# sashajenner/honours

Hardware: AMD Instinct MI355X
Metric: raw-signal MB/s (compress+decompress) (higher is better)
Workload: dtype u16

## Files before the change

honours_amd/csrc/press_huffman.hip:

```cpp

#include "press_internal.h"
#include "press_packed.h"
#include <cstddef>
#include <type_traits>

namespace ph {

#ifdef HUF_STAMPS
__device__ unsigned long long g_hstamp[32];
#define HSTAMP_DECL                                             \
	unsigned long long hs_t = __builtin_amdgcn_s_memtime(); \
	unsigned long long hs_acc[8] = { 0, 0, 0, 0, 0, 0, 0, 0 }
#define HSTAMP(i)                                                              \
	do {     \
		__builtin_amdgcn_sched_barrier(0);                             \
		const unsigned long long hs_n = __builtin_amdgcn_s_memtime(); \
		hs_acc[(i) & 7] += hs_n - hs_t;                                \
		hs_t = hs_n;                                                   \
		__builtin_amdgcn_sched_barrier(0);                             \
	} while (0)
#define HSTAMP_FLUSH(base)                                                     \
	do {                                                                   \
		if ((threadIdx.x & 63) == 0)                                   \
			for (int hs_i = 0; hs_i < 8; hs_i++)                   \
// ... 54 lines not shown
	typedef uint32_t u32x4_u __attribute__((ext_vector_type(4), aligned(1)));
	const u32x4_u v = __builtin_nontemporal_load(reinterpret_cast<const u32x4_u *>(p));
	return make_uint4(v.x, v.y, v.z, v.w);
}
__device__ __forceinline__ uint32_t ld4_pay(const uint8_t *p)
{
	typedef uint32_t __attribute__((aligned(1))) u32_u;
	return __builtin_nontemporal_load(reinterpret_cast<const u32_u *>(p));
}
#else
__device__ __forceinline__ uint4 ld16_pay(const uint8_t *p)
{
	uint4 v;
	__builtin_memcpy(&v, p, 16);
	return v;
}
__device__ __forceinline__ uint32_t ld4_pay(const uint8_t *p)
{
	uint32_t v;
	__builtin_memcpy(&v, p, 4);
	return v;
}
#endif

template <int NDW, int S = 64>
__device__ __forceinline__ void col_load(uint32_t *col, const uint8_t *src, int32_t rb0, int32_t lo, int32_t nby)
{
	if (rb0 >= lo && rb0 + 4 * NDW <= nby) {
		const uint8_t *q = src + rb0;
		uint4 t[NDW / 4 ? NDW / 4 : 1];
		uint32_t x[NDW % 4 ? NDW % 4 : 1];
#pragma unroll
		for (int j = 0; j < NDW / 4; j++)
			t[j] = ld16_pay(q + 16 * j);
#pragma unroll
		for (int j = 0; j < NDW % 4; j++)
			x[j] = ld4_pay(q + 4 * (NDW / 4 * 4 + j));
#pragma unroll
		for (int j = 0; j < NDW / 4; j++) {
			col[(4 * j + 0) * S] = t[j].x;
			col[(4 * j + 1) * S] = t[j].y;
			col[(4 * j + 2) * S] = t[j].z;
			col[(4 * j + 3) * S] = t[j].w;
		}
#pragma unroll
		for (int j = 0; j < NDW % 4; j++)
			col[(NDW / 4 * 4 + j) * S] = x[j];
	} else if (nby > lo) {
		uint8_t b[4 * NDW];
#pragma unroll
		for (int i = 0; i < 4 * NDW; i++) {
			const int32_t r = rb0 + i;
			b[i] = src[r < lo ? lo : (r >= nby ? nby - 1 : r)];
		}
#pragma unroll
		for (int j = 0; j < NDW; j++) {
			uint32_t x = 0;
#pragma unroll
			for (int i = 0; i < 4; i++) {
				const int32_t r = rb0 + 4 * j + i;
				x |= (r >= lo && r < nby) ? (uint32_t) b[4 * j + i] << (8 * i) : 0u;
			}
			col[j * S] = x;
		}
	} else {
#pragma unroll
		for (int j = 0; j < NDW; j++)
			col[j * S] = 0;
	}
}

__device__ __forceinline__ int32_t unzz8(uint32_t z) { return (int32_t) (z >> 1) ^ -(int32_t) (z & 1u); }

typedef __attribute__((address_space(3))) const uint32_t *lds_cu32p;
typedef __attribute__((address_space(3))) const uint16_t *lds_cu16p;
typedef __attribute__((address_space(3))) const uint8_t *lds_cu8p;
typedef __attribute__((address_space(3))) uint8_t *lds_u8p;

struct LenTabs {
	alignas(16) uint32_t alut[1 << HUF_LUT_BITS];
	alignas(16) uint16_t flut[1 << HUF_LUT_BITS];
	alignas(16) uint16_t l2ld[HUF_L2_ENTRIES];
};

template <bool TRIE, int S = 64>
__device__ __forceinline__ uint32_t len_scan(const uint32_t *col_, const LenTabs *tabs, const HuffDev *hd, uint32_t start,
					     uint32_t lim, uint32_t nb, uint32_t &cnt, uint32_t &dsum)
{
	const lds_cu32p col = (lds_cu32p) col_;
	const lds_cu32p alut = (lds_cu32p) tabs->alut;
	const lds_cu16p flut = (lds_cu16p) tabs->flut;
	const lds_cu16p l2ld = (lds_cu16p) tabs->l2ld;
	bool bad = start == HEND;
	uint32_t L = lim < nb ? lim : nb;
	if (bad)
		L = 0;
	auto long_ld = [&](uint32_t e, uint32_t wnd) -> uint32_t {
		if (TRIE && e == 0xFFFFFFFFu) {
			const uint32_t t = trie_code(hd, wnd);
			return t ? (((t >> 24) & 31u) | (((uint32_t) unzz8(t & 0xFFu) & 0xFFu) << 8)) : 0u;
		}
		const uint32_t v = l2ld[(e & 0xFFFu) + ((wnd >> HUF_LUT_BITS) & ((1u << ((e >> 12) & 15u)) - 1u))];
		return v == 0xFFFFu ? 0u : v;
	};
	constexpr uint32_t PB = 30;
	const lds_cu32p colm = col - S;
	uint32_t A = (bad ? 0u : start) + PB;
	{
		int32_t LmP = (int32_t) L - HUF_LUT_BITS + (int32_t) PB;
		uint32_t jj = (A >> 5) & 15u;
		uint32_t w0 = colm[__umul24(jj, (uint32_t) S)], w1 = colm[__umul24(jj, (uint32_t) S) + S];
		while ((int32_t) (A & 0x1FFu) <= LmP) {
			const uint32_t pp = A & 0x1FFu;
			{
				const uint32_t w2 = colm[__umul24(jj, (uint32_t) S) + 2 * S];
				const uint32_t wnd = __builtin_amdgcn_alignbit(w1, w0, A);
				const uint32_t e = *(lds_cu32p) ((lds_cu8p) alut + (wnd & (((1u << HUF_LUT_BITS) - 1u) << 2)));
				uint32_t inc = e;
				if ((int32_t) e < 0) {
					const uint32_t ld = long_ld(e, wnd >> 2);
					const uint32_t tot = ld & 0xFFu;
					inc = tot | (1u << HUF_A_CNT) | (((uint32_t) (int32_t) (int8_t) (ld >> 8) & 0x7FFFu) << HUF_A_SUM);
					if (tot - 1u >= L + PB - pp) {
						inc = 0;
						LmP = -1;
					}
				}
				A += inc;
				const uint32_t jn = (A >> 5) & 15u;
				if (jn != jj) {
					w0 = w1;
					w1 = w2;
				}
				jj = jn;
			}
		}
	}
	uint32_t p = (A & 0x1FFu) - PB;
	uint32_t c = (A >> HUF_A_CNT) & 0x7Fu;
	int32_t d = (int32_t) (A << 1) >> 17;
	for (;;) {
		const bool act = p < L;
		if (!any64(act))
			break;
		const uint32_t pp = act ? p : 0u;
		const uint32_t j = pp >> 5;
		const int r0 = (int) __umul24(j, (uint32_t) S);
		const uint32_t wnd = __builtin_amdgcn_alignbit(col[r0 + S], col[r0], pp);
		const uint32_t e = alut[wnd & ((1u << HUF_LUT_BITS) - 1u)];
		const uint32_t f = flut[wnd & ((1u << HUF_LUT_BITS) - 1u)];
		uint32_t tot = e & 15u, n = (e >> HUF_A_CNT) & 15u, len1 = f & 0xFFu;
		int32_t dall = (int32_t) (e << 1) >> 17, d1 = (int32_t) (int8_t) (f >> 8);
		bool fail = false;
		if (any64(act && (int32_t) e < 0)) {
			if (act && (int32_t) e < 0) {
				const uint32_t ld = long_ld(e, wnd);
				tot = len1 = ld & 0xFFu;
				dall = d1 = (int32_t) (int8_t) (ld >> 8);
				fail = tot == 0;
				n = 1;
			}
		}
		const bool fits = pp + tot <= L;
		const bool cut = !fits && pp + len1 > nb;
		if (act && !fail && !cut) {
			p += fits ? tot : len1;
			c += fits ? n : 1u;
			d += fits ? dall : d1;
		}
		if (act && (fail || cut)) {
			bad = true;
			L = 0;
		}
	}
	cnt = c;
	dsum = (uint32_t) d & 0xFFFFu;
	return bad ? HEND : (p >= nb && p < lim ? HEND : p);
}

__device__ __forceinline__ void wave_lds_sync()
{
	__builtin_amdgcn_fence(__ATOMIC_RELEASE, "wavefront");
	__builtin_amdgcn_wave_barrier();
	__builtin_amdgcn_fence(__ATOMIC_ACQUIRE, "wavefront");
}



#ifndef HUF_SYNC_PER_CU
#define HUF_SYNC_PER_CU 2
#endif
#ifndef HUF_RUNUP_EIGHTHS
#define HUF_RUNUP_EIGHTHS 4
#endif
constexpr int WGS = 1024;
constexpr int SYNC_S = 64;

__device__ __forceinline__ uint32_t pack_rec(uint32_t f, uint32_t c, uint32_t d)
{
	return (f == HEND ? R_END : f) | ((c & 0xFFu) << 8) | ((d & 0xFFFFu) << 16);
}

constexpr uint32_t LIST_NONE = 0xFFFFFFFFu;
constexpr uint32_t SYNC_UC = 16;

__device__ __forceinline__ void list_push(uint32_t *list, uint32_t *cnt, uint32_t cap, bool yes, uint32_t value, uint32_t lane)
{
	const unsigned long long m = __ballot(yes);
// ... 336 lines not shown
		if (e < nex)
			val[e] = z | (((xcum + before + inc - dl) & 0xFFFFu) << 16);
		xcum += total;
		__syncthreads();
	}
	__syncthreads();
	const uint64_t cumall = s_cum;
	const uint32_t nlow = cumall < want ? (uint32_t) cumall : want;
	const bool fused = nlow >= 1 && (nex == 0 || pos[nex - 1] < nlow + nex);
	const uint32_t zd0 = uniform(a.meta[r].zd0) & 0xFFFFu, q = uniform(a.meta[r].q);
	const uint64_t src0 = a.htiles[k0].src;
	const int64_t nby0 = (int64_t) ((a.htiles[k0].nbits + 7u) >> 3);
	uint64_t cum = 0;
	uint32_t dcum = 0;
	for (uint32_t b = 0; b < nu; b += HT) {
		const uint32_t u = b + tid;
		uint32_t c = 0, dt = 0;
		if (u < nu) {
			const uint2 w = hw[u];
			c = w.x;
			dt = w.y & 0xFFFFu;
		}
		const uint32_t inc = wave_scan(c);
		const uint32_t dinc = wave_scan(dt);
		if ((tid & 63) == 63) {
			s_w[tid >> 6] = inc;
			s_wd[tid >> 6] = dinc;
		}
		__syncthreads();
		uint32_t before = 0, total = 0, dbefore = 0, dtotal = 0;
#pragma unroll
		for (int w2 = 0; w2 < HT / 64; w2++) {
			const uint32_t x = s_w[w2], y = s_wd[w2];
			if (w2 < (int) (tid >> 6)) {
				before += x;
				dbefore += y;
			}
			total += x;
			dtotal += y;
		}
		if (u < nu) {
			const uint64_t ob = cum + before + inc - c;
			const uint32_t L0 = ob > 0xFFFFFFFFull ? 0xFFFFFFFFu : (uint32_t) ob;
			const uint32_t quota = L0 >= want ? 0u : (c < want - L0 ? c : want - L0);
			const uint32_t L1 = L0 + quota;
			uint32_t Ea = 0, Eb = 0;
			if (fused && quota) {
				keys_below2(pos, nex, L0, L1, Ea, Eb);
				if (L1 == nlow)
					Eb = nex;
			}
			uint32_t bz = zd0;
			if (L0) {
				bz = unzz16(zd0) + ((dcum + dbefore + dinc - dt) & 0xFFFFu);
				if (Ea) {
					const uint32_t pv = val[Ea - 1];
					bz += (pv >> 16) + unzz16(pv & 0xFFFFu);
				}
				bz &= 0xFFFFu;
			}
			const uint64_t src = src0 + (uint64_t) u * UB;
			const int64_t nby = nby0 - (int64_t) u * UB;
			const uint32_t nbyc = nby <= 0 ? 0u : (nby > (int64_t) HUF_U_NBY ? HUF_U_NBY : (uint32_t) nby);
			uint4 *d = reinterpret_cast<uint4 *>(a.hunit + (uint64_t) k0 * UPT + u);
			d[0] = make_uint4((uint32_t) src, (uint32_t) (src >> 32) | (bz << 16), (uint32_t) o0, (uint32_t) (o0 >> 32));
			d[1] = make_uint4(L0, quota | (nbyc << 14) | ((q & 15u) << 26) | (fused ? 1u << 30 : 0u), Ea, Eb - Ea);
		}
		cum += total;
		dcum += dtotal;
		__syncthreads();
	}
	static_assert(HUF_U_QUOTA >= 64u * 255u, "a unit's quota");
	if (tid == 0) {
		a.meta[r].nlow = nlow;
		if (fused)
			a.hread[2 * r + 1] = nt | HUF_FUSED;
	}
}


constexpr uint32_t EMIT_STG = 4096;

template <bool TRIE>
__device__ __forceinline__ void emit_codes(const uint32_t *col_, const uint32_t *lut_, const uint16_t *lut2_,
					   const HuffDev *hd, uint32_t p, uint32_t nmine, uint8_t *wp_)
{
	const lds_cu32p col = (lds_cu32p) col_;
	const lds_cu8p lut = (lds_cu8p) lut_;
	const lds_cu16p lut2 = (lds_cu16p) lut2_;
	auto long_entry = [&](uint32_t e, uint32_t wnd) -> uint32_t {
		if (TRIE && e == 0xFFFFFFFFu) {
			const uint32_t t = trie_code(hd, wnd);
			return t ? ((t & 0xFFFFFF00u) | ((uint32_t) unzz8(t & 0xFFu) & 0xFFu)) : 0u;
		}
		const uint32_t e2 = lut2[(e & 0xFFFu) + ((wnd >> HUF_LUT_BITS) & ((1u << ((e >> 12) & 15u)) - 1u))];
		return e2 == 0xFFFFu ? 0u : (((uint32_t) unzz8(e2 & 0xFFu) & 0xFFu) | (e2 & 0x1F00u) | ((e2 & 0x1F00u) << 16));
	};
	typedef lds_u8p WP;
	WP w = (WP) wp_;
	const WP wend = w + nmine;
	WP wlim = nmine ? wend - 1 : w;
	constexpr uint32_t PB = 30;
	const lds_cu32p colm = col - 64;
	uint32_t pp = p + PB;
	uint32_t jj = pp >> 5;
	uint32_t w0 = colm[__umul24(jj, 64u)], w1 = colm[__umul24(jj, 64u) + 64];
	while (w < wlim) {
		{
			const uint32_t w2 = colm[__umul24(jj, 64u) + 128];
			const uint32_t wnd = __builtin_amdgcn_alignbit(w1, w0, pp);
			uint32_t e = *(lds_cu32p) (lut + (wnd & (((1u << HUF_LUT_BITS) - 1u) << 2)));
			if (e >= HUF_LONG)
				e = long_entry(e, wnd >> 2);
			w[0] = (uint8_t) e;
			w[1] = (uint8_t) (e >> 16);
			w += 1u + ((e >> 29) & 1u);
			pp += (e >> 8) & 0x1Fu;
			const uint32_t jn = pp >> 5;
			if (jn != jj) {
				w0 = w1;
				w1 = w2;
			}
			jj = jn;
		}
	}
	if (w < wend) {
		const uint32_t wnd = __builtin_amdgcn_alignbit(w1, w0, pp);
		uint32_t e = *(lds_cu32p) (lut + (wnd & (((1u << HUF_LUT_BITS) - 1u) << 2)));
		if (e >= HUF_LONG)
			e = long_entry(e, wnd >> 2);
		w[0] = (uint8_t) e;
	}
}


__device__ __forceinline__ uint32_t lower_bound_u32(const uint32_t *p, uint32_t n, uint32_t key)
{
	uint32_t lo = 0, hi = n;
	while (lo < hi) {
		const uint32_t mid = (lo + hi) >> 1;
		if (p[mid] < key)
			lo = mid + 1;
		else
			hi = mid;
	}
	return lo;
}

template <typename LOWAT>
__device__ __forceinline__ void gather8(LOWAT lowat, const uint32_t *pos, const uint32_t *val, uint32_t zd0,
					uint32_t i0, uint32_t Ia, uint32_t Ib, uint32_t e_first, uint32_t e_cnt,
					uint32_t v[4])
{
	v[0] = v[1] = v[2] = v[3] = 0;
	const uint32_t lo = i0 > Ia ? i0 : Ia;
	const uint32_t hi = i0 + 8 < Ib ? i0 + 8 : Ib;
	if (lo >= hi)
		return;
	const uint32_t uf = lo ? lo - 1 : 0;
	const uint32_t e_end = e_first + e_cnt;
	uint32_t e = e_first + lower_bound_u32(pos + e_first, e_cnt, uf);
	uint32_t l = uf - e;
	uint32_t nextpos = e < e_end ? pos[e] : 0xFFFFFFFFu;
#pragma unroll
	for (int h = 0; h < 8; h++) {
		const uint32_t i = i0 + h;
		if (i >= lo && i < hi) {
			uint32_t dl;
			if (i == 0) {
				dl = unzz16(zd0);
			} else if (i - 1 == nextpos) {
				dl = unzz16(val[e] & 0xFFFFu);
				e++;
				nextpos = e < e_end ? pos[e] : 0xFFFFFFFFu;
			} else {
				dl = lowat(l) & 0xFFFFu;
				l++;
			}
			v[h >> 1] |= dl << (16 * (h & 1));
		}
	}
}

struct EmitRead {
	const uint32_t *pos, *val;
	int16_t *out;
	uint32_t zd0, q;
};

constexpr uint32_t EMIT_ALIGN = 8;

__device__ __forceinline__ void expand8s(uint2 dd, uint32_t v[4])
{
	typedef short i16x2 __attribute__((ext_vector_type(2)));
	const i16x2 eight = { 8, 8 };
	const uint32_t t[4] = { __builtin_amdgcn_perm(0, dd.x, 0x010c000c), __builtin_amdgcn_perm(0, dd.x, 0x030c020c),
				__builtin_amdgcn_perm(0, dd.y, 0x010c000c), __builtin_amdgcn_perm(0, dd.y, 0x030c020c) };
#pragma unroll
	for (int h = 0; h < 4; h++)
		v[h] = __builtin_bit_cast(uint32_t, __builtin_bit_cast(i16x2, t[h]) >> eight);
}

struct EmitPlan {
	uint32_t L0, L1;
	uint32_t Ea, ecnt;
	uint32_t Ia, Ib;
	uint32_t base;
	uint32_t pe;
};

__device__ __forceinline__ void emit_samples16(const uint8_t *src, const EmitRead &R, const EmitPlan &P, uint32_t lane)
{
	const uint32_t L0 = P.L0, L1 = P.L1, Ea = P.Ea, ecnt = P.ecnt, Ia = P.Ia, Ib = P.Ib, pe = P.pe;
// ... 28 lines not shown
					const uint64_t m = lo >= 8 ? 0ull : ~((1ull << (8 * lo)) - 1ull);
					dd.x &= (uint32_t) m;
					dd.y &= (uint32_t) (m >> 32);
				};
				mask8(da, i0);
				mask8(db, i0 + 8);
			}
			expand8s(da, v);
			expand8s(db, v + 4);
		} else {
			auto lowat = [&](uint32_t l) -> uint32_t { return (l >= L0 && l < L1) ? (uint32_t) (int32_t) (int8_t) src[l - L0] : 0u; };
			gather8(lowat, R.pos, R.val, R.zd0, i0, Ia, Ib, Ea, ecnt, v);
			gather8(lowat, R.pos, R.val, R.zd0, i0 + 8, Ia, Ib, Ea, ecnt, v + 4);
			__builtin_amdgcn_s_waitcnt(0x0F70);
		}
		const uint32_t ta = lane_prefix8(v) & 0xFFFFu;
		const uint32_t tb = lane_prefix8(v + 4) & 0xFFFFu;
		const uint32_t tot = (ta + tb) & 0xFFFFu;
		const uint32_t inc = wave_incl_scan_dpp(tot);
		const uint32_t ba = (base + inc - tot) & 0xFFFFu, bb = (ba + ta) & 0xFFFFu;
		const uint32_t ba2 = ba | (ba << 16), bb2 = bb | (bb << 16);
#pragma unroll
		for (int h = 0; h < 4; h++) {
			v[h] = pk_add16(v[h], ba2);
			v[4 + h] = pk_add16(v[4 + h], bb2);
		}
		if (shift) {
#pragma unroll
			for (int h = 0; h < 8; h++)
				v[h] = __builtin_bit_cast(uint32_t, __builtin_bit_cast(u16x2, v[h]) << qq);
		}
#if defined(EMIT_ABL) && EMIT_ABL == 1
		if (R.q == 0x7FFFFFFFu)
#endif
#pragma unroll
		for (int hh = 0; hh < 2; hh++) {
			const uint32_t ia = i0 + 8 * hh;
			if (!ragged || (ia >= Ia && ia + 8 <= Ib)) {
				typedef uint32_t u32x4 __attribute__((ext_vector_type(4)));
				const u32x4 vv = { v[4 * hh], v[4 * hh + 1], v[4 * hh + 2], v[4 * hh + 3] };
#ifdef EMIT_NT_STORES
				__builtin_nontemporal_store(vv, reinterpret_cast<u32x4 *>(R.out + ia));
#else
				*reinterpret_cast<u32x4 *>(R.out + ia) = vv;
#endif
			} else if (ia < Ib && ia + 8 > Ia) {
#pragma unroll
				for (uint32_t h = 0; h < 8; h++)
					if (ia + h >= Ia && ia + h < Ib)
						R.out[ia + h] = (int16_t) (v[4 * hh + (h >> 1)] >> (16 * (h & 1)));
			}
		}
		base += (uint32_t) __builtin_amdgcn_readlane((int) inc, 63);
	}
}

__device__ __forceinline__ uint32_t zz_bytes(uint32_t d)
{
	return ((d << 1) & 0xFEFEFEFEu) ^ (((d >> 7) & 0x01010101u) * 0xFFu);
}

#ifndef EMIT_WG
#define EMIT_WG 512
#endif
#ifndef EMIT_PER_CU
#define EMIT_PER_CU 2
#endif
constexpr int WGE = EMIT_WG;
constexpr uint32_t EMIT_UC = 16;

struct EmitStg {
	uint8_t pre[16];
	uint8_t s[WGE / 64][EMIT_STG];
	uint8_t post[32];
};

template <int RU, bool TRIE>
__global__ __launch_bounds__(WGE) void k_huf_emit(DecodeArgs a)
{
	constexpr int OWN = HufGeo<RU>::OWN, NDW = HufGeo<RU>::NDW, NCOL = HufGeo<RU>::NDW;
	constexpr uint32_t EW = WGE / 64;
	struct Lds {
		alignas(16) uint32_t lut[1 << HUF_LUT_BITS];
		alignas(16) uint16_t lut2[HUF_L2_ENTRIES];
		uint32_t img[EW][NCOL * 64];
		uint32_t pad_row[2 * 64];
		alignas(16) EmitStg stg_all;
	};
	__shared__ __attribute__((aligned(16))) Lds lds;
	auto &lut = lds.lut;
	auto &lut2 = lds.lut2;
	auto &img = lds.img;
	auto &pad_row = lds.pad_row;
	auto &stg_all = lds.stg_all;
	__shared__ unsigned long long s_chunk[64];
	__shared__ uint32_t s_ticket;

	const uint32_t lane = threadIdx.x & 63;
	const uint32_t wv = threadIdx.x >> 6;
	const uint32_t ntiles = min(uniform(a.ctl->nchunks), a.max_htiles);
	const uint32_t nunits = ntiles * (HT / 64);
	if (threadIdx.x == 0) {
		pad_row[0] = 0;
		s_ticket = 0;
	}
	if (threadIdx.x < 64)
		s_chunk[threadIdx.x] = ~0ull;
	{
		const uint4 *s4 = reinterpret_cast<const uint4 *>(a.huff->lut32);
		uint4 *d4 = reinterpret_cast<uint4 *>(lut);
		for (uint32_t i = threadIdx.x; i < (1u << HUF_LUT_BITS) / 4; i += WGE)
			d4[i] = s4[i];
		const uint4 *t4 = reinterpret_cast<const uint4 *>(a.huff->lut2);
		uint4 *u4 = reinterpret_cast<uint4 *>(lut2);
		for (uint32_t i = threadIdx.x; i < (uint32_t) HUF_L2_ENTRIES / 8; i += WGE)
			u4[i] = t4[i];
	}
	uint32_t *col = img[wv] + lane;
	uint8_t *stg = stg_all.s[wv];
	__syncthreads();
	auto draw = [&]() -> uint32_t {
		uint32_t u = 0;
		if (lane == 0) {
			const uint32_t t = atomicAdd(&s_ticket, 1u);
			const uint32_t c = t / EMIT_UC, slot = t % EMIT_UC;
			unsigned long long *cs = &s_chunk[c & 63u];
			if (slot == 0) {
				u = atomicAdd(&a.ctl->units, EMIT_UC);
				__hip_atomic_store(cs, ((unsigned long long) c << 32) | u, __ATOMIC_RELAXED, __HIP_MEMORY_SCOPE_WORKGROUP);
			} else {
				unsigned long long v;
				do {
					v = __hip_atomic_load(cs, __ATOMIC_RELAXED, __HIP_MEMORY_SCOPE_WORKGROUP);
				} while ((uint32_t) (v >> 32) != c);
				u = (uint32_t) v + slot;
			}
		}
		return uniform(u);
	};
	static_assert(offsetof(HufUnit, obase) == 16 && offsetof(HufUnit, ecnt) == 28, "the plan is read as eight dwords");
	static_assert(63 * (OWN / 8) + 4 * NDW <= HUF_U_NBY, "HufUnit::qnf's byte count tells whether every lane's bytes lie inside");
	auto fetch_unit = [&](uint32_t u) -> uint32_t {
		uint32_t v = 0;
		if (u < nunits && lane < 8)
			v = reinterpret_cast<const uint32_t *>(a.hunit + u)[lane];
		return v;
	};
	struct Unit {
		uint32_t u, obase, quota, nby, fused, q, bz, ea, ecnt;
		uint64_t srco, roff;
	};
	auto resolve = [&](uint32_t u, uint32_t tv) -> Unit {
		auto at = [&](int i) -> uint32_t { return (uint32_t) __builtin_amdgcn_readlane((int) tv, i); };
		Unit U;
		U.u = u;
		const uint32_t hb = at(1), qnf = at(5);
		U.srco = ((uint64_t) (hb & 0xFFFFu) << 32) | at(0);
		U.bz = hb >> 16;
		U.roff = ((uint64_t) at(3) << 32) | at(2);
		U.obase = at(4);
		U.quota = qnf & HUF_U_QUOTA;
		U.nby = (qnf >> 14) & HUF_U_NBY;
		U.q = (qnf >> 26) & 15u;
		U.fused = qnf >> 30;
		U.ea = at(6);
		U.ecnt = at(7);
		return U;
	};
	struct Stage2 {
		uint32_t pay[NDW];
		uint32_t rec, pe;
		bool fast;
	};
	auto issue2 = [&](const Unit &U, Stage2 &S) {
		const int32_t rb0 = (int32_t) lane * (OWN / 8);
		S.fast = U.nby >= 63 * (OWN / 8) + 4 * NDW;
		const uint8_t *q = a.in + U.srco + rb0;
		if (S.fast) {
			uint4 t[NDW / 4 ? NDW / 4 : 1];
#pragma unroll
			for (int j = 0; j < NDW / 4; j++)
				t[j] = ld16_pay(q + 16 * j);
#pragma unroll
			for (int j = 0; j < NDW % 4; j++)
				S.pay[NDW / 4 * 4 + j] = ld4_pay(q + 4 * (NDW / 4 * 4 + j));
#pragma unroll
			for (int j = 0; j < NDW / 4; j++) {
				S.pay[4 * j + 0] = t[j].x;
				S.pay[4 * j + 1] = t[j].y;
				S.pay[4 * j + 2] = t[j].z;
				S.pay[4 * j + 3] = t[j].w;
			}
		}
		S.rec = a.hrec[(uint64_t) U.u * 64 + lane];
		S.pe = (U.ecnt <= 64 && lane < U.ecnt) ? a.ex_pos[U.roff + U.ea + lane] : 0xFFFFFFFFu;
	};
	auto land2 = [&](const Unit &U, const Stage2 &S) {
		wave_lds_sync();
		if (S.fast) {
#pragma unroll
			for (int j = 0; j < NDW; j++)
				col[j * 64] = S.pay[j];
		} else {
			col_load<NDW>(col, a.in + U.srco, (int32_t) lane * (OWN / 8), 0, (int32_t) U.nby);
		}
		wave_lds_sync();
	};
	HSTAMP_DECL;
	const uint32_t u_first = draw();
	if (u_first >= nunits)
		return;
	Unit U = resolve(u_first, fetch_unit(u_first)), Un = {}, Unn = {};
	Stage2 S, Sn = {};
	issue2(U, S);
	land2(U, S);
	uint32_t u_nxt = draw();
	if (u_nxt < nunits)
		Un = resolve(u_nxt, fetch_unit(u_nxt));
	for (;;) {
		const uint32_t u_nn = draw();
		const uint32_t tv_nn = fetch_unit(u_nn);
		const bool more = u_nxt < nunits;
		if (more)
			issue2(Un, Sn);
		HSTAMP(0);
		const uint32_t rec = S.rec;
		const uint32_t quota = U.quota;
		const uint32_t obase = U.obase;
		const uint64_t roff = U.roff;
		const uint32_t cnt = (rec >> 8) & 0xFFu;
		const uint32_t inc = wave_scan(cnt);
		const bool fused = U.fused != 0;
		const uint32_t ex = inc - cnt;
		const uint32_t f = rec & 0xFFu;
		const uint32_t p0 = f == R_END ? 0u : f;
		uint32_t nmine = (ex >= quota || f == R_END) ? 0u : (cnt < quota - ex ? cnt : quota - ex);
		nmine = ex >= EMIT_STG ? 0u : (nmine < EMIT_STG - ex ? nmine : EMIT_STG - ex);
		HSTAMP(2);
		{
#if defined(EMIT_ABL) && EMIT_ABL == 3
			if (a.nreads == 0x7FFFFFFFu)
#endif
			emit_codes<TRIE>(col, lut, lut2, a.huff, p0, nmine, stg + ex);
			HSTAMP(3);
			const uint32_t pe = S.pe;
			if (more)
				land2(Un, Sn);
			else
				wave_lds_sync();
			if (u_nn < nunits)
				Unn = resolve(u_nn, tv_nn);
			HSTAMP(1);
			if (fused) {
				if (quota) {
					EmitRead R;
					R.pos = a.ex_pos + roff;
					R.val = a.ex_val + roff;
					R.out = a.sig + roff;
					R.zd0 = U.bz;
					R.q = U.q;
					EmitPlan P;
					P.L0 = obase;
					P.L1 = obase + quota;
					P.Ea = U.ea;
					P.ecnt = U.ecnt;
					P.Ia = obase ? obase + U.ea + 1 : 0u;
					P.Ib = P.L1 + U.ea + U.ecnt + 1;
					P.base = obase ? U.bz : 0u;
					P.pe = pe;
					HSTAMP(4);
#if defined(EMIT_ABL) && EMIT_ABL == 2
					if (a.nreads == 0x7FFFFFFFu)
#endif
					emit_samples16(stg, R, P, lane);
					HSTAMP(5);
				}
			} else {
				uint8_t *dst = a.low + roff + obase;
				for (uint32_t o = lane * 16; o < quota; o += 64 * 16) {
					uint4 v = *reinterpret_cast<const uint4 *>(stg + o);
					v = make_uint4(zz_bytes(v.x), zz_bytes(v.y), zz_bytes(v.z), zz_bytes(v.w));
					if (o + 16 <= quota) {
						__builtin_memcpy(dst + o, &v, 16);
					} else {
						const uint32_t vv[4] = { v.x, v.y, v.z, v.w };
						for (uint32_t b = 0; o + b < quota; b++)
							dst[o + b] = (uint8_t) (vv[b >> 2] >> (8 * (b & 3)));
					}
				}
			}
			wave_lds_sync();
		}
		HSTAMP(6);
		if (!more)
			break;
		U = Un;
		S = Sn;
		Un = Unn;
		u_nxt = u_nn;
	}
	HSTAMP_FLUSH(8);
}


constexpr uint32_t TILES_RPW = 16;
__global__ __launch_bounds__(64) void k_huff_tiles(DecodeArgs a)
{
	const uint32_t lane = threadIdx.x;
	const uint32_t r = lane < TILES_RPW ? blockIdx.x * TILES_RPW + lane : 0xFFFFFFFFu;
	const uint32_t minlen = a.huff->minlen, maxlen = a.huff->maxlen;
	const uint32_t OWN = minlen >= 4 ? 256u : minlen >= 2 ? 128u : 64u;
	const uint64_t TB = (uint64_t) HT * OWN;
	uint32_t nt = 0;
	if (r < a.nreads && a.meta[r].status == 0) {
		const ReadMeta *m = a.meta + r;
		const uint32_t hdr = m->hdr + m->seclen + 4;
		const uint64_t nbytes64 = a.in_len[r] - hdr;
		const uint64_t nbits = 8ull * (nbytes64 > 0x1FFFFFFFull ? 0x1FFFFFFFull : nbytes64);
		const uint64_t need = (uint64_t) m->nlow * maxlen;
		const uint64_t span = nbits < need ? nbits : need;
		nt = (uint32_t) ((span + TB - 1) / TB);
	}
	uint32_t inc = nt;
#pragma unroll
	for (int dd = 1; dd < 64; dd <<= 1) {
		const uint32_t t2 = (uint32_t) __shfl_up((int) inc, dd, 64);
// ... 110 lines not shown
```

honours_amd/csrc/press_internal.h:

```cpp
#pragma once

#include <hip/hip_runtime.h>
#include <stdint.h>

namespace ph {

enum ExFmt : int {
	EXF_VBE21 = 0,
	EXF_VBBE21 = 1,
	EXF_VBSBE21 = 2,
	EXF_VBSSE21 = 3,
	EXF_EXZD = 4
};

struct ReadMeta {
	uint32_t nex;
	uint32_t ored;
	uint32_t zd0;
	uint32_t q;
	uint32_t hdr;
	uint32_t seclen;
	uint32_t nlow;
	uint32_t status;
};

constexpr int HUF_LUT_BITS = 12;
constexpr int HUF_L2_ENTRIES = 3072;
constexpr int HUF_L2_IDS = 64;
struct HuffDev {
	uint32_t enc[256];
	uint16_t lut[1 << HUF_LUT_BITS];
	int16_t child[1024][2];
	int16_t leaf[1024];
	uint32_t minlen, maxlen;
	uint16_t lut2[HUF_L2_ENTRIES];
	uint16_t l2off[256];
	uint8_t l2bits[256];
	alignas(16) uint32_t lut32[1 << HUF_LUT_BITS];
	alignas(16) uint32_t mlut[1 << HUF_LUT_BITS];
	alignas(16) uint16_t l2ld[HUF_L2_ENTRIES];
	alignas(16) uint32_t alut[1 << HUF_LUT_BITS];
	alignas(16) uint16_t flut[1 << HUF_LUT_BITS];
};
constexpr uint32_t HUF_A_CNT = 9, HUF_A_SUM = 16;
constexpr uint32_t HUF_NEEDS_TRIE = 0x80000000u;
constexpr uint32_t HUF_L2_NONE = HUF_L2_ENTRIES - 1;
constexpr uint32_t HUF_MLONG = 1u << 31;
constexpr uint32_t HUF_M_MAXN = 8;
constexpr uint32_t HUF_LONG = 1u << 30;
constexpr uint32_t HUF_TWO = 1u << 29;

constexpr int HUF_HT = 256;
struct HufUnit {
	uint32_t src_lo;
	uint32_t src_hi_bz;
	uint64_t roff;
	uint32_t obase;
	uint32_t qnf;
	uint32_t ea, ecnt;
};
static_assert(sizeof(HufUnit) == 32, "HufUnit");
constexpr uint32_t HUF_U_QUOTA = 0x3FFFu, HUF_U_NBY = 0xFFFu;
constexpr uint32_t HUF_FUSED = 0x80000000u;

constexpr uint32_t CHUNK = 32768;
struct ChunkDesc {
	uint64_t sig_off;
	uint64_t out_base;
	uint32_t n;
	uint32_t j;
	uint32_t read;
	uint32_t cap_ok;
	uint64_t ebefore;
	uint32_t ecnt[4];
	uint16_t kmask[4];
};
static_assert(sizeof(ChunkDesc) == 64, "ChunkDesc is one 64-byte line");
struct ChunkBits {
	uint64_t before;
	uint32_t q[4];
	uint32_t pad[2];
};
struct ChunkCtl {
	uint32_t ticket;
	uint32_t pad0[31];
	uint32_t nchunks;
	uint32_t pad1[31];
	uint32_t ticket2;
	uint32_t pad2[31];
	uint32_t lists[32];
	uint32_t units;
	uint32_t pad4[31];
	uint32_t sunits;
	uint32_t pad5[31];
};

struct BatchArgs {
	const int16_t *sig;
	const uint64_t *off;
	const uint32_t *nsamp;
	uint8_t *out;
	const uint64_t *out_off;
	uint64_t *out_len;
	ReadMeta *meta;
	uint32_t *ex_pos;
	uint32_t *ex_val;
	const HuffDev *huff;
	uint32_t nreads;
	ChunkDesc *chunks;
	uint64_t *gran;
	ChunkCtl *ctl;
	uint32_t max_chunks;
	ChunkBits *cbits;
	uint8_t *low_tmp;
	uint32_t *first_chunk;
	uint32_t *zhist;
	uint32_t *zkcnt;
};

struct HufTile {
	uint64_t src;
	uint64_t low;
	uint32_t nbits;
	uint32_t t_last;
	uint32_t read;
	uint32_t want;
};

struct DecodeArgs {
	const uint8_t *in;
	const uint64_t *in_off;
	const uint64_t *in_len;
	int16_t *sig;
// ... 147 lines not shown
```

honours_amd/csrc/press_table.hip:

```cpp

#include <stdlib.h>

#include <vector>

#include "press_host.h"

using namespace ph;

static inline int32_t unzz8(uint32_t z) { return (int32_t) (z >> 1) ^ -(int32_t) (z & 1u); }

int ph::upload_table(const uint32_t len[256], const uint64_t bits[256])
{
	if (g.have_table && !memcmp(len, g.tlen, sizeof g.tlen) && !memcmp(bits, g.tbits, sizeof g.tbits))
		return 0;
	std::vector<HuffDev> hv(1);
	HuffDev &h = hv[0];
	memset(&h, 0xFF, sizeof h);
	int nnodes = 1, ncoded = 0;
	bool needs_trie = false;
	for (int s = 0; s < 256; s++) {
		const uint32_t l = len[s];
		if (l > 24)
			return set_error(PRESS_HIP_EARG, "Huffman table: symbol %d has a code of %u bits (at most 24)", s, l);
		if (l == 0) {
			h.enc[s] = 0;
			continue;
		}
		ncoded++;
		h.enc[s] = (uint32_t) (bits[s] & 0xFFFFFFu) | (l << 24);
		int p = 0;
		for (uint32_t k = 0; k < l; k++) {
			const int b = (int) ((bits[s] >> k) & 1);
			if (h.leaf[p] >= 0)
				return set_error(PRESS_HIP_EARG, "Huffman table: not a prefix code");
			if (h.child[p][b] < 0) {
				if (nnodes >= 1024)
					return set_error(PRESS_HIP_EARG, "Huffman table: too many nodes");
				h.child[p][b] = (int16_t) nnodes++;
			}
			p = h.child[p][b];
		}
		if (h.child[p][0] >= 0 || h.child[p][1] >= 0)
			return set_error(PRESS_HIP_EARG, "Huffman table: not a prefix code");
		h.leaf[p] = (int16_t) s;
		if (l <= (uint32_t) HUF_LUT_BITS) {
			const uint32_t step = 1u << l;
			for (uint32_t i = (uint32_t) bits[s] & (step - 1); i < (1u << HUF_LUT_BITS); i += step)
				h.lut[i] = (uint16_t) (s | (l << 8));
		}
	}
	{
		int nid = 0;
		uint32_t used = 0;
		int id_of[1 << HUF_LUT_BITS];
		for (int i = 0; i < (1 << HUF_LUT_BITS); i++)
			id_of[i] = -1;
		uint32_t depth[256] = { 0 };
		int prefix_of[256];
		for (int s = 0; s < 256; s++) {
			if (len[s] <= (uint32_t) HUF_LUT_BITS)
				continue;
			const int pfx = (int) (bits[s] & ((1u << HUF_LUT_BITS) - 1));
			if (id_of[pfx] < 0 && nid < HUF_L2_IDS) {
				prefix_of[nid] = pfx;
				id_of[pfx] = nid++;
			}
			if (id_of[pfx] >= 0 && len[s] - HUF_LUT_BITS > depth[id_of[pfx]])
				depth[id_of[pfx]] = len[s] - HUF_LUT_BITS;
		}
		for (uint32_t d = 32; d >= 1; d--) {
			for (int id = 0; id < nid; id++) {
				if (depth[id] != d)
					continue;
				if (d > 12 || used + (1u << d) > (uint32_t) HUF_L2_ENTRIES)
					continue;
				h.l2off[id] = (uint16_t) used;
				h.l2bits[id] = (uint8_t) d;
				h.lut[prefix_of[id]] = (uint16_t) (0x8000u | (uint32_t) id);
				used += 1u << d;
			}
		}
		for (int s = 0; s < 256; s++) {
			if (len[s] <= (uint32_t) HUF_LUT_BITS)
				continue;
			const int pfx = (int) (bits[s] & ((1u << HUF_LUT_BITS) - 1));
			const int id = id_of[pfx];
			if (id < 0 || h.lut[pfx] != (uint16_t) (0x8000u | (uint32_t) id))
				continue;
			const uint32_t rest = (uint32_t) (bits[s] >> HUF_LUT_BITS), rl = len[s] - HUF_LUT_BITS;
			for (uint32_t i = rest; i < (1u << depth[id]); i += 1u << rl)
				h.lut2[h.l2off[id] + i] = (uint16_t) (s | (len[s] << 8));
		}
		needs_trie = used > HUF_L2_NONE;
		for (int s = 0; s < 256; s++) {
			if (len[s] <= (uint32_t) HUF_LUT_BITS)
				continue;
			const int pfx = (int) (bits[s] & ((1u << HUF_LUT_BITS) - 1));
			const int id = id_of[pfx];
			if (id < 0 || h.lut[pfx] != (uint16_t) (0x8000u | (uint32_t) id))
				needs_trie = true;
		}
		for (int i = 0; i < HUF_L2_ENTRIES; i++) {
			const uint32_t e2 = h.lut2[i];
			h.l2ld[i] = e2 == 0xFFFFu ? (uint16_t) 0xFFFFu : (uint16_t) ((e2 >> 8) | ((unzz8(e2 & 0xFFu) & 0xFFu) << 8));
		}
	}
	for (uint32_t i = 0; i < (1u << HUF_LUT_BITS); i++) {
		const uint16_t e1 = h.lut[i];
		if (e1 == 0xFFFFu) {
			h.lut32[i] = needs_trie ? 0xFFFFFFFFu : (HUF_LONG | HUF_L2_NONE);
		} else if (e1 & 0x8000u) {
			const uint32_t id = e1 & 0xFFu;
			h.lut32[i] = HUF_LONG | ((uint32_t) h.l2bits[id] << 12) | h.l2off[id];
		} else {
			const uint32_t s1 = (uint32_t) unzz8(e1 & 0xFFu) & 0xFFu, l1 = e1 >> 8;
			uint32_t v = s1 | (l1 << 8) | (l1 << 24);
			const uint32_t rest = (uint32_t) HUF_LUT_BITS - l1;
			const uint16_t e2 = h.lut[i >> l1];
			if (e2 != 0xFFFFu && !(e2 & 0x8000u) && (uint32_t) (e2 >> 8) <= rest)
				v = s1 | ((l1 + (e2 >> 8)) << 8) | (((uint32_t) unzz8(e2 & 0xFFu) & 0xFFu) << 16) | (l1 << 24) | HUF_TWO;
			h.lut32[i] = v;
		}
	}
	for (uint32_t i = 0; i < (1u << HUF_LUT_BITS); i++) {
		uint32_t pos = 0, n = 0, len1 = 0;
		int32_t d1 = 0, dsum = 0;
		for (;;) {
			const uint16_t e1 = h.lut[i >> pos];
			if (e1 == 0xFFFFu || (e1 & 0x8000u) || pos + (uint32_t) (e1 >> 8) > (uint32_t) HUF_LUT_BITS)
				break;
			const int32_t d = (int32_t) unzz8(e1 & 0xFFu);
			if (!n) {
				len1 = e1 >> 8;
				d1 = d;
			}
			dsum += d;
			pos += e1 >> 8;
			n++;
			if (pos == (uint32_t) HUF_LUT_BITS || n == HUF_M_MAXN)
				break;
		}
		const uint16_t e0 = h.lut[i];
		if (n)
			h.mlut[i] = pos | (n << 4) | (len1 << 8) | (((uint32_t) d1 & 0xFFu) << 12) | (((uint32_t) dsum & 0x7FFu) << 20);
		else if (e0 != 0xFFFFu && (e0 & 0x8000u))
			h.mlut[i] = HUF_MLONG | (uint32_t) h.l2off[e0 & 0xFFu] | ((uint32_t) h.l2bits[e0 & 0xFFu] << 12);
		else
			h.mlut[i] = needs_trie ? 0xFFFFFFFFu : (HUF_MLONG | HUF_L2_NONE);
		h.alut[i] = n ? (pos | (n << HUF_A_CNT) | (((uint32_t) dsum & 0x7FFFu) << HUF_A_SUM)) : h.mlut[i];
		h.flut[i] = n ? (uint16_t) (len1 | (((uint32_t) d1 & 0xFFu) << 8)) : (uint16_t) 0;
	}
	if (!ncoded)
		return set_error(PRESS_HIP_EARG, "Huffman table: no symbol has a code");
	h.minlen = 64;
	h.maxlen = 0;
	for (int s = 0; s < 256; s++) {
		if (!len[s])
			continue;
		h.minlen = len[s] < h.minlen ? len[s] : h.minlen;
		h.maxlen = len[s] > h.maxlen ? len[s] : h.maxlen;
	}
	if (g.huff.reserve(sizeof(HuffDev)))
		return PRESS_HIP_EHIP;
	HIPCHK(hipMemcpy(g.huff.p, &h, sizeof h, hipMemcpyHostToDevice));
	memcpy(g.tlen, len, sizeof g.tlen);
	memcpy(g.tbits, bits, sizeof g.tbits);
	g.tmin = h.minlen;
	g.tmax = h.maxlen;
	g.table_trie = needs_trie;
	g.have_table = true;
	return 0;
}

namespace {
int parse_table_file(FILE *fp, uint32_t len[256], uint64_t bits[256]);
}

extern "C" int press_hip_set_table(const uint32_t len[256], const uint64_t bits[256])
{
	API_ENTER;
	return upload_table(len, bits);
}

extern "C" int press_hip_load_table_file(const char *path)
{
	uint32_t len[256];
	uint64_t bits[256];
	FILE *fp = fopen(path, "rb");
	if (!fp)
		return set_error(PRESS_HIP_EARG, "cannot open %s", path);
	int rc = parse_table_file(fp, len, bits);
	fclose(fp);
	if (rc)
		return rc;
	return press_hip_set_table(len, bits);
}


namespace {

huffman_node *new_node(bool leaf, unsigned char sym)
{
	huffman_node *p = (huffman_node *) calloc(1, sizeof *p);
	if (!p)
		return nullptr;
	p->isLeaf = leaf ? 1 : 0;
	if (leaf)
		p->symbol = sym;
	return p;
}

int parse_table_file(FILE *fp, uint32_t len[256], uint64_t bits[256])
{
	unsigned char hd[8];
	memset(len, 0, 256 * sizeof len[0]);
	memset(bits, 0, 256 * sizeof bits[0]);
	if (fread(hd, 1, 8, fp) != 8)
		return set_error(PRESS_HIP_EARG, "Huffman table: short header");
	uint32_t count = ((uint32_t) hd[0] << 24) | ((uint32_t) hd[1] << 16) | ((uint32_t) hd[2] << 8) | hd[3];
	if (count > 256)
		return set_error(PRESS_HIP_EARG, "Huffman table: %u entries", count);
	for (uint32_t i = 0; i < count; i++) {
		int sym = fgetc(fp), nb = fgetc(fp);
		if (sym == EOF || nb == EOF || nb == 0 || nb > 64)
			return set_error(PRESS_HIP_EARG, "Huffman table: bad entry %u", i);
		unsigned char code[8] = { 0 };
		if (fread(code, 1, (size_t) (nb + 7) / 8, fp) != (size_t) (nb + 7) / 8)
			return set_error(PRESS_HIP_EARG, "Huffman table: truncated");
		uint64_t b = 0;
		for (int k = 0; k < nb; k++)
			if (code[k / 8] & (1u << (k % 8)))
				b |= 1ull << k;
// ... 150 lines not shown
```

Baseline: 795,100.

## Fold second-level Huffman lookups into the main LUT load as deferred iterations

Re-encodes long-code LUT entries to carry a byte offset into a second-level table placed contiguously after the primary LUT in LDS. In both the length scan and the emit loop, a long code now stores a pending address and resolves it on the next loop iteration through the same single LDS load, instead of taking a divergent branch with a separate lookup. The emit path stores a new precomputed 32-bit second-level table so entries can be used directly. This removes branch divergence on rare long codes, at the cost of an extra loop iteration per long code and a larger LDS footprint in the emit kernel.

After: 752,500. -5.4%, worse.

```diff
diff --git a/honours_amd/csrc/press_huffman.hip b/honours_amd/csrc/press_huffman.hip
--- a/honours_amd/csrc/press_huffman.hip
+++ b/honours_amd/csrc/press_huffman.hip
@@ -160,6 +160,7 @@
 	alignas(16) uint16_t flut[1 << HUF_LUT_BITS];
 	alignas(16) uint16_t l2ld[HUF_L2_ENTRIES];
 };
+static_assert(offsetof(LenTabs, alut) == 0 && offsetof(LenTabs, l2ld) == HUF_A_L2, "alut's long entries hold l2ld's place behind it");
 
 template <bool TRIE, int S = 64>
 __device__ __forceinline__ uint32_t len_scan(const uint32_t *col_, const LenTabs *tabs, const HuffDev *hd, uint32_t start,
@@ -168,7 +169,6 @@
 	const lds_cu32p col = (lds_cu32p) col_;
 	const lds_cu32p alut = (lds_cu32p) tabs->alut;
 	const lds_cu16p flut = (lds_cu16p) tabs->flut;
-	const lds_cu16p l2ld = (lds_cu16p) tabs->l2ld;
 	bool bad = start == HEND;
 	uint32_t L = lim < nb ? lim : nb;
 	if (bad)
@@ -178,7 +178,7 @@
 			const uint32_t t = trie_code(hd, wnd);
 			return t ? (((t >> 24) & 31u) | (((uint32_t) unzz8(t & 0xFFu) & 0xFFu) << 8)) : 0u;
 		}
-		const uint32_t v = l2ld[(e & 0xFFFu) + ((wnd >> HUF_LUT_BITS) & ((1u << ((e >> 12) & 15u)) - 1u))];
+		const uint32_t v = *(lds_cu16p) ((lds_cu8p) alut + ((e >> HUF_L2_AT) & 0x7FFFu) + (__builtin_amdgcn_ubfe(wnd, HUF_LUT_BITS, e & 15u) << 1));
 		return v == 0xFFFFu ? 0u : v;
 	};
 	constexpr uint32_t PB = 30;
@@ -188,20 +188,35 @@
 		int32_t LmP = (int32_t) L - HUF_LUT_BITS + (int32_t) PB;
 		uint32_t jj = (A >> 5) & 15u;
 		uint32_t w0 = colm[__umul24(jj, (uint32_t) S)], w1 = colm[__umul24(jj, (uint32_t) S) + S];
+		uint32_t l2a = 0;
 		while ((int32_t) (A & 0x1FFu) <= LmP) {
 			const uint32_t pp = A & 0x1FFu;
 			{
 				const uint32_t w2 = colm[__umul24(jj, (uint32_t) S) + 2 * S];
 				const uint32_t wnd = __builtin_amdgcn_alignbit(w1, w0, A);
-				const uint32_t e = *(lds_cu32p) ((lds_cu8p) alut + (wnd & (((1u << HUF_LUT_BITS) - 1u) << 2)));
+				const uint32_t a1 = wnd & (((1u << HUF_LUT_BITS) - 1u) << 2);
+				const uint32_t l2d = l2a & 0x7FFCu;
+				const uint32_t e = *(lds_cu32p) ((lds_cu8p) alut + (a1 > l2d ? a1 : l2d));
 				uint32_t inc = e;
-				if ((int32_t) e < 0) {
-					const uint32_t ld = long_ld(e, wnd >> 2);
+				if ((int32_t) (e | l2a) < 0) {
+					const bool pend = (int32_t) l2a < 0;
+					uint32_t ld = __builtin_amdgcn_ubfe(e, (l2a & 2u) << 3, 16);
+					bool got = pend;
+					if (TRIE && !pend && e == 0xFFFFFFFFu) {
+						ld = long_ld(e, wnd >> 2);
+						got = true;
+					}
+					ld = ld == 0xFFFFu ? 0u : ld;
 					const uint32_t tot = ld & 0xFFu;
 					inc = tot | (1u << HUF_A_CNT) | (((uint32_t) (int32_t) (int8_t) (ld >> 8) & 0x7FFFu) << HUF_A_SUM);
-					if (tot - 1u >= L + PB - pp) {
+					if (got && tot - 1u >= L + PB - pp) {
 						inc = 0;
 						LmP = -1;
+					}
+					l2a = 0;
+					if (!got) {
+						inc = 0;
+						l2a = HUF_MLONG | (((e >> HUF_L2_AT) & 0x7FFFu) + (__builtin_amdgcn_ubfe(wnd, HUF_LUT_BITS + 2, e & 15u) << 1));
 					}
 				}
 				A += inc;
@@ -704,19 +719,17 @@
 constexpr uint32_t EMIT_STG = 4096;
 
 template <bool TRIE>
-__device__ __forceinline__ void emit_codes(const uint32_t *col_, const uint32_t *lut_, const uint16_t *lut2_,
-					   const HuffDev *hd, uint32_t p, uint32_t nmine, uint8_t *wp_)
+__device__ __forceinline__ void emit_codes(const uint32_t *col_, const uint32_t *lut_, const HuffDev *hd, uint32_t p,
+					   uint32_t nmine, uint8_t *wp_)
 {
 	const lds_cu32p col = (lds_cu32p) col_;
 	const lds_cu8p lut = (lds_cu8p) lut_;
-	const lds_cu16p lut2 = (lds_cu16p) lut2_;
-	auto long_entry = [&](uint32_t e, uint32_t wnd) -> uint32_t {
-		if (TRIE && e == 0xFFFFFFFFu) {
-			const uint32_t t = trie_code(hd, wnd);
-			return t ? ((t & 0xFFFFFF00u) | ((uint32_t) unzz8(t & 0xFFu) & 0xFFu)) : 0u;
-		}
-		const uint32_t e2 = lut2[(e & 0xFFFu) + ((wnd >> HUF_LUT_BITS) & ((1u << ((e >> 12) & 15u)) - 1u))];
-		return e2 == 0xFFFFu ? 0u : (((uint32_t) unzz8(e2 & 0xFFu) & 0xFFu) | (e2 & 0x1F00u) | ((e2 & 0x1F00u) << 16));
+	auto trie_entry = [&](uint32_t wnd) -> uint32_t {
+		const uint32_t t = trie_code(hd, wnd);
+		return t ? ((t & 0x1FFFFF00u) | ((uint32_t) unzz8(t & 0xFFu) & 0xFFu) | HUF_ONE) : HUF_ONE;
+	};
+	auto l2_slot = [&](uint32_t e, uint32_t wnd) -> uint32_t {
+		return ((e >> HUF_L2_AT) & 0x7FFFu) + (__builtin_amdgcn_ubfe(wnd, HUF_LUT_BITS + 2, e & 15u) << 2);
 	};
 	typedef lds_u8p WP;
 	WP w = (WP) wp_;
@@ -727,16 +740,21 @@
 	uint32_t pp = p + PB;
 	uint32_t jj = pp >> 5;
 	uint32_t w0 = colm[__umul24(jj, 64u)], w1 = colm[__umul24(jj, 64u) + 64];
+	bool pend = false;
+	uint32_t l2a = 0;
 	while (w < wlim) {
 		{
 			const uint32_t w2 = colm[__umul24(jj, 64u) + 128];
 			const uint32_t wnd = __builtin_amdgcn_alignbit(w1, w0, pp);
-			uint32_t e = *(lds_cu32p) (lut + (wnd & (((1u << HUF_LUT_BITS) - 1u) << 2)));
-			if (e >= HUF_LONG)
-				e = long_entry(e, wnd >> 2);
+			const uint32_t a1 = wnd & (((1u << HUF_LUT_BITS) - 1u) << 2);
+			uint32_t e = *(lds_cu32p) (lut + (pend ? l2a : a1));
+			if (TRIE && e == 0xFFFFFFFFu)
+				e = trie_entry(wnd >> 2);
 			w[0] = (uint8_t) e;
 			w[1] = (uint8_t) (e >> 16);
-			w += 1u + ((e >> 29) & 1u);
+			pend = (int32_t) e < 0;
+			l2a = l2_slot(e, wnd);
+			w += (e >> 29) & 3u;
 			pp += (e >> 8) & 0x1Fu;
 			const uint32_t jn = pp >> 5;
 			if (jn != jj) {
@@ -749,8 +767,10 @@
 	if (w < wend) {
 		const uint32_t wnd = __builtin_amdgcn_alignbit(w1, w0, pp);
 		uint32_t e = *(lds_cu32p) (lut + (wnd & (((1u << HUF_LUT_BITS) - 1u) << 2)));
-		if (e >= HUF_LONG)
-			e = long_entry(e, wnd >> 2);
+		if (TRIE && e == 0xFFFFFFFFu)
+			e = trie_entry(wnd >> 2);
+		else if ((int32_t) e < 0)
+			e = *(lds_cu32p) (lut + l2_slot(e, wnd));
 		w[0] = (uint8_t) e;
 	}
 }
@@ -945,14 +965,15 @@
 	constexpr uint32_t EW = WGE / 64;
 	struct Lds {
 		alignas(16) uint32_t lut[1 << HUF_LUT_BITS];
-		alignas(16) uint16_t lut2[HUF_L2_ENTRIES];
+		alignas(16) uint32_t lut2e[HUF_L2_ENTRIES];
 		uint32_t img[EW][NCOL * 64];
 		uint32_t pad_row[2 * 64];
 		alignas(16) EmitStg stg_all;
 	};
 	__shared__ __attribute__((aligned(16))) Lds lds;
 	auto &lut = lds.lut;
-	auto &lut2 = lds.lut2;
+	auto &lut2e = lds.lut2e;
+	static_assert(offsetof(Lds, lut2e) - offsetof(Lds, lut) == HUF_E_L2, "lut32's long entries hold lut2e's place behind it");
 	auto &img = lds.img;
 	auto &pad_row = lds.pad_row;
 	auto &stg_all = lds.stg_all;
@@ -974,9 +995,9 @@
 		uint4 *d4 = reinterpret_cast<uint4 *>(lut);
 		for (uint32_t i = threadIdx.x; i < (1u << HUF_LUT_BITS) / 4; i += WGE)
 			d4[i] = s4[i];
-		const uint4 *t4 = reinterpret_cast<const uint4 *>(a.huff->lut2);
-		uint4 *u4 = reinterpret_cast<uint4 *>(lut2);
-		for (uint32_t i = threadIdx.x; i < (uint32_t) HUF_L2_ENTRIES / 8; i += WGE)
+		const uint4 *t4 = reinterpret_cast<const uint4 *>(a.huff->lut2e);
+		uint4 *u4 = reinterpret_cast<uint4 *>(lut2e);
+		for (uint32_t i = threadIdx.x; i < (uint32_t) HUF_L2_ENTRIES / 4; i += WGE)
 			u4[i] = t4[i];
 	}
 	uint32_t *col = img[wv] + lane;
@@ -1104,7 +1125,7 @@
 #if defined(EMIT_ABL) && EMIT_ABL == 3
 			if (a.nreads == 0x7FFFFFFFu)
 #endif
-			emit_codes<TRIE>(col, lut, lut2, a.huff, p0, nmine, stg + ex);
+			emit_codes<TRIE>(col, lut, a.huff, p0, nmine, stg + ex);
 			HSTAMP(3);
 			const uint32_t pe = S.pe;
 			if (more)
diff --git a/honours_amd/csrc/press_internal.h b/honours_amd/csrc/press_internal.h
--- a/honours_amd/csrc/press_internal.h
+++ b/honours_amd/csrc/press_internal.h
@@ -37,6 +37,7 @@
 	uint16_t l2off[256];
 	uint8_t l2bits[256];
 	alignas(16) uint32_t lut32[1 << HUF_LUT_BITS];
+	alignas(16) uint32_t lut2e[HUF_L2_ENTRIES];
 	alignas(16) uint32_t mlut[1 << HUF_LUT_BITS];
 	alignas(16) uint16_t l2ld[HUF_L2_ENTRIES];
 	alignas(16) uint32_t alut[1 << HUF_LUT_BITS];
@@ -47,8 +48,12 @@
 constexpr uint32_t HUF_L2_NONE = HUF_L2_ENTRIES - 1;
 constexpr uint32_t HUF_MLONG = 1u << 31;
 constexpr uint32_t HUF_M_MAXN = 8;
-constexpr uint32_t HUF_LONG = 1u << 30;
-constexpr uint32_t HUF_TWO = 1u << 29;
+constexpr uint32_t HUF_LONG = 1u << 31;
+constexpr uint32_t HUF_ONE = 1u << 29, HUF_TWO = 2u << 29;
+constexpr uint32_t HUF_E_L2 = 4u << HUF_LUT_BITS;
+constexpr uint32_t HUF_A_L2 = (4u + 2u) << HUF_LUT_BITS;
+constexpr uint32_t HUF_L2_AT = 14;
+static_assert(HUF_E_L2 + 4u * HUF_L2_ENTRIES <= 1u << 15 && HUF_A_L2 + 2u * HUF_L2_ENTRIES <= 1u << 15, "a long entry's offset field");
 
 constexpr int HUF_HT = 256;
 struct HufUnit {
diff --git a/honours_amd/csrc/press_table.hip b/honours_amd/csrc/press_table.hip
--- a/honours_amd/csrc/press_table.hip
+++ b/honours_amd/csrc/press_table.hip
@@ -103,18 +103,19 @@
 		for (int i = 0; i < HUF_L2_ENTRIES; i++) {
 			const uint32_t e2 = h.lut2[i];
 			h.l2ld[i] = e2 == 0xFFFFu ? (uint16_t) 0xFFFFu : (uint16_t) ((e2 >> 8) | ((unzz8(e2 & 0xFFu) & 0xFFu) << 8));
+			h.lut2e[i] = e2 == 0xFFFFu ? HUF_ONE : (((uint32_t) unzz8(e2 & 0xFFu) & 0xFFu) | (e2 & 0x1F00u) | ((e2 & 0x1F00u) << 16) | HUF_ONE);
 		}
 	}
 	for (uint32_t i = 0; i < (1u << HUF_LUT_BITS); i++) {
 		const uint16_t e1 = h.lut[i];
 		if (e1 == 0xFFFFu) {
-			h.lut32[i] = needs_trie ? 0xFFFFFFFFu : (HUF_LONG | HUF_L2_NONE);
+			h.lut32[i] = needs_trie ? 0xFFFFFFFFu : (HUF_LONG | ((HUF_E_L2 + 4u * HUF_L2_NONE) << HUF_L2_AT));
 		} else if (e1 & 0x8000u) {
 			const uint32_t id = e1 & 0xFFu;
-			h.lut32[i] = HUF_LONG | ((uint32_t) h.l2bits[id] << 12) | h.l2off[id];
+			h.lut32[i] = HUF_LONG | ((HUF_E_L2 + 4u * h.l2off[id]) << HUF_L2_AT) | h.l2bits[id];
 		} else {
 			const uint32_t s1 = (uint32_t) unzz8(e1 & 0xFFu) & 0xFFu, l1 = e1 >> 8;
-			uint32_t v = s1 | (l1 << 8) | (l1 << 24);
+			uint32_t v = s1 | (l1 << 8) | (l1 << 24) | HUF_ONE;
 			const uint32_t rest = (uint32_t) HUF_LUT_BITS - l1;
 			const uint16_t e2 = h.lut[i >> l1];
 			if (e2 != 0xFFFFu && !(e2 & 0x8000u) && (uint32_t) (e2 >> 8) <= rest)
@@ -147,7 +148,10 @@
 			h.mlut[i] = HUF_MLONG | (uint32_t) h.l2off[e0 & 0xFFu] | ((uint32_t) h.l2bits[e0 & 0xFFu] << 12);
 		else
 			h.mlut[i] = needs_trie ? 0xFFFFFFFFu : (HUF_MLONG | HUF_L2_NONE);
-		h.alut[i] = n ? (pos | (n << HUF_A_CNT) | (((uint32_t) dsum & 0x7FFFu) << HUF_A_SUM)) : h.mlut[i];
+		h.alut[i] = n ? (pos | (n << HUF_A_CNT) | (((uint32_t) dsum & 0x7FFFu) << HUF_A_SUM))
+			      : h.mlut[i] == 0xFFFFFFFFu
+				      ? 0xFFFFFFFFu
+				      : (HUF_MLONG | ((HUF_A_L2 + 2u * (h.mlut[i] & 0xFFFu)) << HUF_L2_AT) | ((h.mlut[i] >> 12) & 15u));
 		h.flut[i] = n ? (uint16_t) (len1 | (((uint32_t) d1 & 0xFFu) << 8)) : (uint16_t) 0;
 	}
 	if (!ncoded)
```
